# nh2/lz4-frame-conduit

Hardware: AMD Instinct MI355X
Metric: GiB/s end-to-end (compress+decompress), 4 MiB blocks, 1/2/4/8 GPUs vs liblz4 (higher is better)
Workload: dtype u8

## Files before the change

### lz4_frame_conduit_amd/csrc/decode_fused.cuh

```cuda
#pragma once
#include "common.cuh"
#include "decode.cuh"

namespace lz4f {

template <int W> struct FzCfg;
template <> struct FzCfg<8> { static constexpr int WAVES = 8; static constexpr uint32_t STAGE = 8192, RING = 8, LDS_BUDGET = 40960; };
template <> struct FzCfg<4> { static constexpr int WAVES = 4; static constexpr uint32_t STAGE = 2048, RING = 4, LDS_BUDGET = 20480; };
struct FzCfgS8 { static constexpr int WAVES = 8; static constexpr uint32_t STAGE = 4096 - 576, RING = 16, LDS_BUDGET = 40960; };
struct FzCfgS4 { static constexpr int WAVES = 4; static constexpr uint32_t STAGE = 2048, RING = 8, LDS_BUDGET = 20480; };
constexpr uint32_t FZ_OVER = 576;
#ifndef FZ_FED_ROUNDS
#define FZ_FED_ROUNDS 1
#endif
#ifndef FZ_STORE_SC1
#define FZ_STORE_SC1 0
#endif
#ifndef FZ_FED_OCC
#define FZ_FED_OCC 8
#endif
constexpr int      FZ_MATCH_SET = 3;
constexpr uint32_t FZ_SRC_BIAS = 1u << 22;
constexpr uint32_t FZ_PEND = 32;
__device__ __forceinline__ bool fz_wait_expired(uint64_t t0, uint64_t budget) { return __builtin_amdgcn_s_memrealtime() - t0 > budget; }

template <class C>
struct alignas(16) FzShared {
    uint4    ring[C::RING][64];
    uint8_t  stage[2][C::STAGE + FZ_OVER];
    uint4    gt[C::WAVES - 1][2][64];
    uint32_t produced;
    uint32_t total_slots;
    uint32_t last_count;
    uint32_t per_slot;
    uint32_t finished;
    uint32_t match_done;
    uint32_t slot_done[C::RING];
    uint32_t slot_cnt[C::RING];
    uint32_t pend_n, prev_ready, own_front;
    uint32_t wait_lo;
    uint32_t pend_dst[FZ_PEND], pend_len[FZ_PEND], pend_off[FZ_PEND];
    int32_t  status;
    uint32_t out_size;
    uint32_t wait_hi;
};
static_assert(sizeof(FzShared<FzCfg<8>>) <= FzCfg<8>::LDS_BUDGET && sizeof(FzShared<FzCfg<4>>) <= FzCfg<4>::LDS_BUDGET, "workgroups per CU");
static_assert(sizeof(FzShared<FzCfgS8>) <= FzCfgS8::LDS_BUDGET && sizeof(FzShared<FzCfgS4>) <= FzCfgS4::LDS_BUDGET, "workgroups per CU");

__device__ __forceinline__ uint32_t lds_peek(const uint32_t* p) { return __atomic_load_n(p, __ATOMIC_RELAXED); }
__device__ __forceinline__ void lds_poke(uint32_t* p, uint32_t v) { __atomic_store_n(p, v, __ATOMIC_RELAXED); }

template <class C>
__device__ __forceinline__ void fz_stage_issue(uint8_t* slot, const uint8_t* __restrict__ in, uint32_t csize, uint32_t s)
{
    const uint32_t lane = lane_id();
    const uint32_t base = s * C::STAGE;
    if (base >= csize) return;
    const uint32_t end = (base + C::STAGE + FZ_OVER < csize) ? base + C::STAGE + FZ_OVER : csize;
    const uint32_t span = end - base;
    for (uint32_t piece = 0; piece < span; piece += 1024) {
        const uint32_t o = piece + lane * 16;
        if (o + 16 <= span) __builtin_amdgcn_global_load_lds((gptr_t)(in + base + o), (lptr_t)(slot + piece), 16, 0, 0);
    }
    const uint32_t tail0 = span & ~15u;
    if (lane < span - tail0) slot[tail0 + lane] = in[base + tail0 + lane];
}

template <class C>
__device__ __forceinline__ void fz_parser(FzShared<C>& sh, const uint8_t* __restrict__ in, uint32_t csize, uint32_t cap, uint64_t hist,
                                          unsigned long long* prof)
{
#ifdef FZ_PROF
    const unsigned long long t_begin = clock64(); unsigned long long t_ring = 0;
#endif
    const uint32_t lane = lane_id();
    uint8_t* stages = &sh.stage[0][0];
    uint32_t nseq = 0, status = 0;
    uint32_t op = 0;
    int32_t  cur = -1;
    uint32_t d0 = 0, d1 = 0, d2 = 0, d3 = 0;

    if (csize == 0) status = 1;
    else fz_stage_issue<C>(stages, in, csize, 0);
    auto need = [&](uint32_t qq) {
        const int32_t s = (int32_t)(qq / C::STAGE);
        if (s == cur) return;
#pragma unroll 1
        for (int32_t it = (s == cur + 1) ? 1 : 0; it < 2; it++) {
            asm volatile("s_waitcnt vmcnt(0)" ::: "memory");
            fz_stage_issue<C>(stages + (uint32_t)((s + it) & 1) * (C::STAGE + FZ_OVER), in, csize, (uint32_t)(s + it));
        }
        cur = s;
    };
    typedef uint32_t v4u_t __attribute__((ext_vector_type(4)));
    v4u_t win = {0u, 0u, 0u, 0u};
    uint32_t wb = 0xFFFFFC00u;
    auto reload = [&](uint32_t qq) {
        need(qq);
        const uint32_t s = qq / C::STAGE;
        const uint32_t o = (qq - s * C::STAGE) & ~7u;
        const uint32_t addr = (uint32_t)(uintptr_t)(lptr_t)(stages + (s & 1) * (C::STAGE + FZ_OVER)) + o + 8u * lane;
        asm volatile("ds_read2_b64 %0, %1 offset1:1\n\ts_waitcnt lgkmcnt(0)" : "=&v"(win) : "v"(addr) : "memory");
        wb = qq & ~7u;
    };
    auto fetch = [&](uint32_t qq) -> uint64_t {
        uint32_t rel = qq - wb;
        if (rel >= 504u) { reload(qq); rel = qq - wb; }
        const uint32_t l = rel >> 3, sh8 = (rel & 7u) * 8u;
        const uint64_t lo = (uint64_t)(uint32_t)__builtin_amdgcn_readlane(win.x, l) | ((uint64_t)(uint32_t)__builtin_amdgcn_readlane(win.y, l) << 32);
        const uint64_t hi = (uint64_t)(uint32_t)__builtin_amdgcn_readlane(win.z, l) | ((uint64_t)(uint32_t)__builtin_amdgcn_readlane(win.w, l) << 32);
        return (lo >> sh8) | ((hi << 1) << (63u - sh8));
    };
    auto ext_slow = [&](uint32_t pos, uint32_t& after) -> uint32_t {
        uint32_t add = 0;
        for (;;) {
            if (pos >= csize || add > 0x7FFF0000u) { status = 1; after = pos; return add; }
            const uint32_t b = uni((uint32_t)in[pos]);
            add += b; pos++;
            if (b != 255) { after = pos; return add; }
        }
    };
    uint32_t v_src = 0, v_lit = 0, v_op = 0, v_ml = 0;
    const uint32_t plog = csize < (96u << 10) ? 3u : 6u, pmask = (1u << plog) - 1u;
    if (lane == 0) sh.per_slot = pmask + 1;
    const uint32_t hist_reach = hist > 65536 ? 65536u : (uint32_t)hist;
    auto finish_slot = [&](uint32_t count) -> bool {
        uint32_t off = 0;
        bool bad = false;
        if (lane < count) {
            const uint64_t room = (uint64_t)cap - v_op;
            if (v_ml) {
                const uint8_t* q = in + v_src + v_lit;
                off = (uint32_t)q[0] | ((uint32_t)q[1] << 8);
                bad = off == 0 || off > v_op + v_lit + hist_reach || (uint64_t)v_lit + v_ml + 5 > room || (uint64_t)v_lit + 12 > room;
            } else bad = v_lit > room;
        }
        d0 = v_src | ((off & 0xFFu) << 24);
        d1 = v_lit | ((off >> 8) << 24);
        d2 = v_op;
        d3 = v_ml;
        return __ballot(bad) == 0;
    };
    auto publish = [&](uint32_t slot_idx) {
#ifdef FZ_PROF
        const unsigned long long tr = clock64();
#endif
        while (slot_idx >= lds_peek(&sh.match_done) + C::RING) __builtin_amdgcn_s_sleep(8);
#ifdef FZ_PROF
        t_ring += clock64() - tr;
#endif
        sh.ring[slot_idx % C::RING][lane] = uint4{d0, d1, d2, d3};
        asm volatile("s_waitcnt lgkmcnt(0)" ::: "memory");
        lds_poke(&sh.produced, slot_idx + 1);
    };
    auto fetch_byte = [&](uint32_t qq) -> uint32_t {
        uint32_t rel = qq - wb;
        if (rel >= 504u) { reload(qq); rel = qq - wb; }
        const uint32_t l = rel >> 3, sh8 = (rel & 7u) * 8u;
        const uint64_t lo = (uint64_t)(uint32_t)__builtin_amdgcn_readlane(win.x, l) | ((uint64_t)(uint32_t)__builtin_amdgcn_readlane(win.y, l) << 32);
        return (uint32_t)(lo >> sh8) & 0xFFu;
    };

    uint32_t pos = 0;
    uint32_t fin = status;
    while (fin == 0) {
        const uint32_t token = fetch_byte(pos);
        uint32_t lit = token >> 4;
        uint32_t p = pos + 1;
        uint32_t bad = 0;
        if (lit == 15) {
            const uint64_t x = fetch(pos) >> 8;
            const uint32_t f = (uint32_t)__builtin_ctzll(~x);
            const uint32_t k = f >> 3;
            lit = 15u + 255u * k + (uint32_t)((x >> (f & 56u)) & 0xFF);
            p = pos + 2 + k;
            if (k == 7) { lit = 15u + ext_slow(pos + 1, p); bad |= status; }
        }
        bad |= p > csize ? 1u : 0u;
        const uint32_t in_left = csize - p;
        const bool is_last = lit > in_left || lit + 8 > in_left || lit + 12 > cap - op;
        uint32_t mlen = 0, npos = pos;
        if (!is_last) {
            const uint32_t qo = p + lit;
            mlen = token & 15;
            npos = qo + 2;
            if (mlen == 15) {
                const uint64_t x = fetch(qo) >> 16;
                const uint32_t f = (uint32_t)__builtin_ctzll(~x);
                const uint32_t k = f >> 3;
                mlen = 15u + 255u * k + (uint32_t)((x >> (f & 56u)) & 0xFF);
                npos = qo + 3 + k;
                if (k == 6) { mlen = 15u + ext_slow(qo + 2, npos); bad |= status; }
                bad |= npos + 4 >= csize ? 1u : 0u;
            }
            mlen += 4;
            bad |= mlen > cap - (op + lit) ? 1u : 0u;
        } else {
            bad |= lit != in_left ? 1u : 0u;
            bad |= lit > cap - op ? 1u : 0u;
        }
        fin |= bad;
        if (fin == 0) {
            const uint32_t slot = nseq & pmask;
            uint32_t keep;
            asm("s_mov_b32 %4, m0\n\ts_mov_b32 m0, %5\n\tv_writelane_b32 %0, %6, m0\n\tv_writelane_b32 %1, %7, m0\n\tv_writelane_b32 %2, %8, m0\n\tv_writelane_b32 %3, %9, m0\n\ts_mov_b32 m0, %4"
                : "+v"(v_src), "+v"(v_lit), "+v"(v_op), "+v"(v_ml), "=&s"(keep) : "s"(slot), "s"(p), "s"(lit), "s"(op), "s"(mlen));
            nseq++;
            op += lit + mlen;
            if (slot == pmask) {
                if (finish_slot(pmask + 1)) publish((nseq >> plog) - 1);
                else { fin |= 1u; nseq -= pmask + 1; }
            }
            pos = npos;
            fin |= is_last ? 2u : (pos >= csize ? 1u : 0u);
        }
    }
    if ((fin & 1u) == 0 && (nseq & pmask) && !finish_slot(nseq & pmask)) fin |= 1u;
    if (fin & 1u) status = 1;
    const uint32_t full = nseq >> plog, part = (status == 0) ? (nseq & pmask) : 0;
    if (part) {
        while (full >= lds_peek(&sh.match_done) + C::RING) __builtin_amdgcn_s_sleep(8);
        sh.ring[full % C::RING][lane] = uint4{d0, d1, d2, d3};
    }
    sh.total_slots = status ? lds_peek(&sh.produced) : full + (part ? 1u : 0u);
    sh.last_count = part ? part : pmask + 1;
    sh.out_size = op;
    sh.status = status ? -1 : 0;
    asm volatile("s_waitcnt lgkmcnt(0)" ::: "memory");
    lds_poke(&sh.finished, 1u);
    if (part) { asm volatile("s_waitcnt lgkmcnt(0)" ::: "memory"); lds_poke(&sh.produced, full + 1); }
#ifdef FZ_PROF
    if (prof && blockIdx.x == 0 && lane == 0) { prof[0] = clock64() - t_begin; prof[1] = t_ring; prof[2] = nseq; }
#endif
}

template <class C>
__device__ __forceinline__ void fz_feeder(FzShared<C>& sh, const SeqDesc* __restrict__ desc, const uint32_t* __restrict__ dsrc, uint32_t nseq,
                                          uint32_t csize, uint32_t cap, uint64_t hist, uint64_t pay_before)
{
    const uint32_t lane = lane_id();
    uint32_t per = (nseq + (C::WAVES - 1) - 1) / (C::WAVES - 1);
    per = per > 64 ? 64u : (per < 8 ? 8u : per);
    const uint32_t nslots = (nseq + per - 1) / per;
    uint32_t expect = 0, status = nseq ? 0u : 1u, published = 0;
    uint4 nxt = {0u, 0u, 0u, 0u};
    uint32_t nxt_src = 0xFFFFFFFFu;
    if (lane < per && lane < nseq) { nxt = ((const uint4*)desc)[lane]; if (dsrc) nxt_src = dsrc[lane]; }
    for (uint32_t slot = 0; slot < nslots && !status; slot++) {
        const uint32_t first = slot * per;
        const uint32_t count = (nseq - first < per) ? nseq - first : per;
        uint4 d = nxt;
        if (nxt_src < (1u << 23) && !(d.w >> 31) && (d.w & 0xFFFFFFu))
            d = uint4{(d.x & 0xFFFFFFu) | ((nxt_src & 0xFFu) << 24), (d.y & 0xFFFFFFu) | (((nxt_src >> 8) & 0xFFu) << 24), d.z,
                      (d.w & 0xFFFFFFu) | 0x80000000u | ((nxt_src >> 16) << 24)};
        const uint32_t nx = first + per + lane;
        nxt = uint4{0u, 0u, 0u, 0u}; nxt_src = 0xFFFFFFFFu;
        if (lane < per && nx < nseq) { nxt = ((const uint4*)desc)[nx]; if (dsrc) nxt_src = dsrc[nx]; }
        const uint32_t p = d.x & 0xFFFFFFu, lit = d.y & 0xFFFFFFu, op = d.z, ml = d.w & 0xFFFFFFu;
        const bool direct = (d.w >> 31) != 0;
        const uint32_t f24 = (d.x >> 24) | ((d.y >> 24) << 8) | (((d.w >> 24) & 0x7Fu) << 16);
        const uint64_t dm = (uint64_t)op + lit, end = dm + ml;
        const uint32_t prev_end = __shfl_up((uint32_t)end, 1);
        const bool last = first + lane + 1 == nseq;
        bool bad = op != (lane == 0 ? expect : prev_end) || (uint64_t)p + lit > csize || end > cap;
        if (last) bad |= ml != 0 || direct;
        else {
            bad |= ml < 4 || end + 5 > cap;
            const int64_t rel = (int64_t)f24 - (int64_t)FZ_SRC_BIAS;
            bad |= direct ? (rel + (int64_t)ml > (int64_t)csize || -rel > (int64_t)pay_before) : (f24 == 0 || f24 > 65535u || f24 > dm + hist);
        }
        if (__ballot(lane < count && bad)) { status = 1; break; }
        expect = __shfl((uint32_t)end, (int)count - 1);
        while (slot >= lds_peek(&sh.match_done) + C::RING && (int32_t)lds_peek((const uint32_t*)&sh.status) >= 0) __builtin_amdgcn_s_sleep(8);
        if ((int32_t)lds_peek((const uint32_t*)&sh.status) < 0) { status = 1; break; }
        sh.ring[slot % C::RING][lane] = d;
        sh.slot_cnt[slot % C::RING] = count;
        if (slot + 1 == nslots) break;
        asm volatile("s_waitcnt lgkmcnt(0)" ::: "memory");
        lds_poke(&sh.produced, slot + 1);
        published = slot + 1;
    }
    sh.total_slots = status ? published : nslots;
    sh.last_count = status ? 64u : nseq - (nslots - 1) * per;
    sh.out_size = expect;
    sh.status = status ? -1 : 0;
    asm volatile("s_waitcnt lgkmcnt(0)" ::: "memory");
    lds_poke(&sh.finished, 1u);
    if (!status) { asm volatile("s_waitcnt lgkmcnt(0)" ::: "memory"); lds_poke(&sh.produced, nslots); }
}

template <class C, bool FED = false>
__device__ __forceinline__ void fz_copier(FzShared<C>& sh, const uint8_t* __restrict__ in, uint8_t* out, uint32_t cw ,
                                          const uint8_t* safe , unsigned long long* prof, const uint32_t* prev_done = nullptr)
{
    const uint32_t lane = lane_id();
    unsigned long long t_wait_p = 0, t_lit = 0, t_wait_m = 0, t_match = 0, n_slots = 0, t_dep = 0, t_drain = 0;
    auto dump = [&]() { if (prof && FED && lane == 0) { atomicAdd(prof + 76, t_wait_p); atomicAdd(prof + 77, t_lit); atomicAdd(prof + 78, t_wait_m); atomicAdd(prof + 79, t_match); }
                        if (prof && blockIdx.x == 0 && lane == 0) { unsigned long long* o = prof + 8 * (cw + 1); o[0] = t_wait_p; o[1] = t_lit; o[2] = t_wait_m; o[3] = t_match; o[4] = n_slots; o[5] = t_dep; o[6] = t_drain; } };
    for (uint32_t slot = cw;; slot += C::WAVES - 1) {
        const unsigned long long c0 = clock64();
        for (;;) {
            if (lds_peek(&sh.produced) > slot) break;
            if (lds_peek(&sh.finished) && slot >= lds_peek(&sh.total_slots)) { dump(); return; }
            __builtin_amdgcn_s_sleep(4);
        }
        const unsigned long long c1 = clock64(); t_wait_p += c1 - c0; n_slots++;
        __builtin_amdgcn_s_setprio(1);
        const uint4 d = sh.ring[slot % C::RING][lane];
        uint32_t count = FED ? 64u : lds_peek(&sh.per_slot);
        if (FED) count = lds_peek(&sh.slot_cnt[slot % C::RING]);
        else if (lds_peek(&sh.finished) && slot + 1 == lds_peek(&sh.total_slots)) count = lds_peek(&sh.last_count);
        count = uni(count);
        const uint32_t vsrc = d.x & 0xFFFFFFu, vlen = d.y & 0xFFFFFFu, vdst = d.z, vml = FED ? (d.w & 0xFFFFFFu) : d.w, voff = (d.x >> 24) | ((d.y >> 24) << 8);
        const bool vdirect = FED && lane < count && (d.w >> 31) != 0;
        const uint32_t vmsrc = (voff | (((d.w >> 24) & 0x7Fu) << 16)) - FZ_SRC_BIAS;

        {
            uint4* T0 = sh.gt[cw][0];
            uint4* T1 = sh.gt[cw][1];
            const uint32_t L = lane < count ? vlen : 0u, M = vdirect ? vml : 0u;
            auto scan = [&](uint32_t v, uint32_t& total) -> uint32_t {
                uint32_t incl = v;
#pragma unroll
                for (int sft = 1; sft < 64; sft <<= 1) { const uint32_t t = __shfl_up(incl, sft); if ((int)lane >= sft) incl += t; }
                total = __builtin_amdgcn_readlane(incl, 63);
                return incl - v;
            };
            auto find = [&](uint32_t u) -> uint32_t {
                uint32_t j = 0;
#pragma unroll
                for (uint32_t step = 32; step; step >>= 1) { const uint32_t c = j + step; if (T0[c].x <= u) j = c; }
                return j;
            };
            uint32_t total;
            {
                const uint32_t uL = L >= 16 ? (L + 15) >> 4 : 0u, uM = M >= 16 ? (M + 15) >> 4 : 0u;
                const uint32_t P = scan(uL + uM, total);
                if (total) {
                    T0[lane] = uint4{P, uL, L, M};
                    T1[lane] = uint4{vsrc, vmsrc, vdst, 0u};
                    __builtin_amdgcn_fence(__ATOMIC_RELEASE, "wavefront"); __builtin_amdgcn_wave_barrier();
                }
            }
            if (total) {
                auto ld = [&](Piece& pc, uint32_t u, uint32_t& dof, bool& act) {
                    const uint32_t j = find(u);
                    const uint4 e0 = T0[j], e1 = T1[j];
                    uint32_t r = u - e0.x;
                    const bool isM = r >= e0.y;
                    r -= isM ? e0.y : 0u;
                    const uint32_t len = isM ? e0.w : e0.z;
                    uint32_t off = r * 16u;
                    off = (off + 16u > len) ? len - 16u : off;
                    act = u < total;
                    dof = e1.z + (isM ? e0.z : 0u) + off;
                    const uint8_t* a = act ? in + (int32_t)((isM ? e1.y : e1.x) + off) : safe;
                    const v4u_ua t = *(const v4u_ua*)a;
                    pc.a = t.a; pc.b = t.b; pc.c = t.c; pc.d = t.d;
                };
                typedef uint32_t u32x4 __attribute__((ext_vector_type(4)));
                typedef u32x4 u32x4_ua __attribute__((aligned(1)));
                auto st = [&](const Piece& pc, uint32_t dof, bool act) {
                    if (!act) return;
#if FZ_STORE_SC1 == 1
                    if (FED) { const u32x4 v = u32x4{pc.a, pc.b, pc.c, pc.d}; uint8_t* q = out + dof; asm volatile("global_store_dwordx4 %0, %1, off sc1\n\ts_nop 1" :: "v"(q), "v"(v) : "memory"); }
#elif FZ_STORE_SC1 == 2
                    if (FED) { const u32x4 v = u32x4{pc.a, pc.b, pc.c, pc.d}; uint8_t* q = out + dof; asm volatile("global_store_dwordx4 %0, %1, off sc0 sc1\n\ts_nop 1" :: "v"(q), "v"(v) : "memory"); }
#elif FZ_STORE_SC1 == 3
                    if (FED) *(v4u_ua*)(out + dof) = v4u_ua{pc.a, pc.b, pc.c, pc.d};
#else
                    if (FED) __builtin_nontemporal_store(u32x4{pc.a, pc.b, pc.c, pc.d}, (u32x4_ua*)(out + dof));
#endif
                    else *(v4u_ua*)(out + dof) = v4u_ua{pc.a, pc.b, pc.c, pc.d};
                };
                constexpr int G = FED ? FZ_FED_ROUNDS : 1;
                Piece pa[G], pb[G];
                uint32_t da[G], db[G];
                bool xa[G], xb[G];
                uint32_t base = 0;
#pragma unroll
                for (int i = 0; i < G; i++) ld(pa[i], base + 64 * i + lane, da[i], xa[i]);
                base += 64 * G;
                for (;;) {
                    const bool more_b = base < total;
#pragma unroll
                    for (int i = 0; i < G; i++) ld(pb[i], base + 64 * i + lane, db[i], xb[i]);
                    base += 64 * G;
#pragma unroll
                    for (int i = 0; i < G; i++) st(pa[i], da[i], xa[i]);
                    if (!more_b) break;
                    const bool more_a = base < total;
#pragma unroll
                    for (int i = 0; i < G; i++) ld(pa[i], base + 64 * i + lane, da[i], xa[i]);
                    base += 64 * G;
#pragma unroll
                    for (int i = 0; i < G; i++) st(pb[i], db[i], xb[i]);
                    if (!more_a) break;
                }
            }
            uint32_t total_b;
            {
                const uint32_t bL = L < 16 ? L : 0u, bM = M < 16 ? M : 0u;
                const uint32_t P = scan(bL + bM, total_b);
                if (total_b) {
                    T0[lane] = uint4{P, bL, L, M};
                    T1[lane] = uint4{vsrc, vmsrc, vdst, 0u};
                    __builtin_amdgcn_fence(__ATOMIC_RELEASE, "wavefront"); __builtin_amdgcn_wave_barrier();
                }
            }
            for (uint32_t base = 0; base < total_b; base += 128) {
                uint8_t v[2]; uint32_t dof[2]; bool act[2];
#pragma unroll
                for (int i = 0; i < 2; i++) {
                    const uint32_t u = base + 64 * i + lane;
                    const uint32_t j = find(u);
                    const uint4 e0 = T0[j], e1 = T1[j];
                    uint32_t r = u - e0.x;
                    const bool isM = r >= e0.y;
                    r -= isM ? e0.y : 0u;
                    act[i] = u < total_b;
                    dof[i] = e1.z + (isM ? e0.z : 0u) + r;
                    const uint8_t* a = act[i] ? in + (int32_t)((isM ? e1.y : e1.x) + r) : safe;
                    v[i] = *a;
                }
#pragma unroll
                for (int i = 0; i < 2; i++) if (act[i]) out[dof[i]] = v[i];
            }
        }
        const unsigned long long c2 = clock64(); t_lit += c2 - c1;
        __builtin_amdgcn_s_setprio(0);
        const uint64_t on_chain = __ballot(lane < count && vml != 0 && !vdirect);
        if (on_chain) {
            while (lds_peek(&sh.match_done) < slot) {
                if ((int32_t)lds_peek((const uint32_t*)&sh.status) < 0) { dump(); return; }
                __builtin_amdgcn_s_sleep(2);
            }
        }
        __builtin_amdgcn_sched_barrier(0); const unsigned long long c3 = clock64(); t_wait_m += c3 - c2; __builtin_amdgcn_sched_barrier(0);
        __builtin_amdgcn_s_setprio(2);
        if (on_chain) {
            constexpr int NJ = FZ_MATCH_SET;
            const uint32_t mdm = vdst + vlen;
            const int32_t ms0 = (int32_t)mdm - (int32_t)voff, ms1 = ms0 + (int32_t)vml;
            const bool has = lane < count && vml != 0 && !vdirect;
            const uint64_t fastmask = __ballot(has && vml >= 16 && vml <= 1024 && voff >= vml);
            uint64_t todo = __ballot(has), unstored = todo;
            uint32_t dep_lo = 0, dep_hi = 0;
            for (uint64_t mm = todo; mm; mm &= mm - 1) {
                const uint32_t k = (uint32_t)__builtin_ctzll(mm);
                const uint32_t dk = __builtin_amdgcn_readlane(mdm, k), mk = __builtin_amdgcn_readlane(vml, k);
                const bool dep = k < lane && ms0 < (int32_t)(dk + mk) && ms1 > (int32_t)dk;
                if (k < 32) dep_lo |= dep ? (1u << k) : 0u; else dep_hi |= dep ? (1u << (k - 32)) : 0u;
            }
            __builtin_amdgcn_sched_barrier(0); t_dep += clock64() - c3; __builtin_amdgcn_sched_barrier(0);
            if (FED && prev_done && lds_peek(&sh.prev_ready) && __ballot(has && ms0 < 0)) __builtin_amdgcn_fence(__ATOMIC_ACQUIRE, "agent");
            if (FED && prev_done && !lds_peek(&sh.prev_ready)) {
                const uint32_t np = lds_peek(&sh.pend_n);
                bool defer = has && ms0 < -(int32_t)lds_peek(&sh.own_front);
                for (uint32_t q = 0; q < np; q++) {
                    const int32_t lo = (int32_t)sh.pend_dst[q], hi = lo + (int32_t)sh.pend_len[q];
                    defer |= has && ms0 < hi && ms1 > lo;
                }
                uint64_t dmask = __ballot(defer);
                while (dmask) {
                    const bool more = has && !defer && (((dep_lo & (uint32_t)dmask) | (dep_hi & (uint32_t)(dmask >> 32))) != 0);
                    const uint64_t add = __ballot(more);
                    if (!add) break;
                    defer |= more; dmask |= add;
                }
                if (dmask) {
                    const uint32_t cnt = (uint32_t)__builtin_popcountll(dmask);
                    if (np + cnt > FZ_PEND) {
                        uint32_t v = 0;
                        const uint64_t budget = (uint64_t)lds_peek(&sh.wait_lo) | ((uint64_t)lds_peek(&sh.wait_hi) << 32);
                        for (const uint64_t t0 = __builtin_amdgcn_s_memrealtime();;) {
                            v = __hip_atomic_load(prev_done, __ATOMIC_RELAXED, __HIP_MEMORY_SCOPE_AGENT);
                            if (v == 1u || v == 2u || fz_wait_expired(t0, budget)) break;
                            __builtin_amdgcn_s_sleep(8);
                        }
                        __builtin_amdgcn_fence(__ATOMIC_ACQUIRE, "agent");
                        if (v != 1u) { lds_poke((uint32_t*)&sh.status, 0xFFFFFFFFu); dump(); return; }
                        for (uint32_t q = 0; q < np; q++) wave_copy_match(out + (int32_t)sh.pend_dst[q], sh.pend_off[q], sh.pend_len[q]);
                        asm volatile("s_waitcnt vmcnt(0)" ::: "memory");
                        lds_poke(&sh.pend_n, 0u);
                        lds_poke(&sh.prev_ready, 1u);
                    } else {
                        if (defer) {
                            const uint32_t at = np + (uint32_t)__builtin_popcountll(dmask & ((1ull << lane) - 1ull));
                            sh.pend_dst[at] = mdm; sh.pend_len[at] = vml; sh.pend_off[at] = voff;
                        }
                        asm volatile("s_waitcnt lgkmcnt(0)" ::: "memory");
                        lds_poke(&sh.pend_n, np + cnt);
                        todo &= ~dmask; unstored &= ~dmask;
                    }
                }
            }
            auto ready = [&]() -> uint64_t {
                return __ballot(has && ((dep_lo & (uint32_t)unstored) | (dep_hi & (uint32_t)(unstored >> 32))) == 0) & todo;
            };
            auto select = [&](CopyJob (&J)[NJ], uint64_t rf) -> uint64_t {
                uint64_t taken = 0;
#pragma unroll
                for (int i = 0; i < NJ; i++) {
                    J[i] = CopyJob{safe, out, 0};
                    if (rf) {
                        const uint32_t c = (uint32_t)__builtin_ctzll(rf);
                        rf &= rf - 1; taken |= 1ull << c;
                        const uint32_t dm = __builtin_amdgcn_readlane(mdm, c);
                        J[i] = CopyJob{out + dm - __builtin_amdgcn_readlane(voff, c), out + dm, (uint32_t)__builtin_amdgcn_readlane(vml, c)};
                    }
                }
                todo &= ~taken;
                return taken;
            };
            while (todo) {
                uint64_t r = ready();
                if ((r & fastmask) == 0) {
                    const uint32_t c = (uint32_t)__builtin_ctzll(r);
                    wave_copy_match(out + __builtin_amdgcn_readlane(mdm, c), __builtin_amdgcn_readlane(voff, c), __builtin_amdgcn_readlane(vml, c));
                    todo &= ~(1ull << c); unstored &= ~(1ull << c);
                    continue;
                }
                CopyJob A[NJ], B[NJ];
                Piece PA[NJ], PB[NJ];
                uint64_t ma = select(A, r & fastmask), mb;
#pragma unroll
                for (int i = 0; i < NJ; i++) job_load(PA[i], A[i], safe);
                for (;;) {
                    mb = select(B, ready() & fastmask);
#pragma unroll
                    for (int i = 0; i < NJ; i++) job_load(PB[i], B[i], safe);
#pragma unroll
                    for (int i = 0; i < NJ; i++) job_store(A[i], PA[i]);
                    unstored &= ~ma;
                    if (mb == 0) break;
                    ma = select(A, ready() & fastmask);
#pragma unroll
                    for (int i = 0; i < NJ; i++) job_load(PA[i], A[i], safe);
#pragma unroll
                    for (int i = 0; i < NJ; i++) job_store(B[i], PB[i]);
                    unstored &= ~mb;
                    if (ma == 0) break;
                }
            }
        }
        __builtin_amdgcn_sched_barrier(0);
        const unsigned long long c5 = clock64();
        __builtin_amdgcn_sched_barrier(0);
        asm volatile("s_waitcnt vmcnt(0)" ::: "memory");
        __builtin_amdgcn_sched_barrier(0);
        t_drain += clock64() - c5;
        __builtin_amdgcn_sched_barrier(0);
        lds_poke(&sh.slot_done[slot % C::RING], slot + 1);
        asm volatile("s_waitcnt lgkmcnt(0)" ::: "memory");
        for (;;) {
            const uint32_t md = lds_peek(&sh.match_done);
            if (lds_peek(&sh.slot_done[md % C::RING]) != md + 1) break;
            if (lane == 0) atomicCAS(&sh.match_done, md, md + 1);
            asm volatile("s_waitcnt lgkmcnt(0)" ::: "memory");
        }
        __builtin_amdgcn_s_setprio(0);
        t_match += clock64() - c3;
    }
}

template <class C, bool FED = false>
__device__ __forceinline__ int32_t fz_decode_block(FzShared<C>& sh, const uint8_t* __restrict__ in, uint32_t csize, uint8_t* out, uint32_t cap, uint64_t hist,
                                                   const uint8_t* safe, unsigned long long* prof, const SeqDesc* __restrict__ fed = nullptr, uint32_t nfed = 0,
                                                   const uint32_t* __restrict__ fed_src = nullptr, uint64_t pay_before = 0, const uint32_t* prev_done = nullptr,
                                                   uint32_t own_front = 0, bool first_of_group = true)
{
    const uint32_t wave = uni(threadIdx.x >> 6);
    __syncthreads();
    if (threadIdx.x == 0) { sh.produced = 0; sh.total_slots = 0; sh.last_count = 64; sh.finished = 0; sh.match_done = 0; sh.status = 0; sh.out_size = 0; }
    if (threadIdx.x < C::RING) sh.slot_done[threadIdx.x] = 0;
    if (threadIdx.x == 0) { if (first_of_group) { sh.pend_n = 0; sh.prev_ready = 0; } sh.own_front = own_front; }
    __syncthreads();
    if (wave == 0) {
        __builtin_amdgcn_s_setprio(3);
        if (FED) fz_feeder<C>(sh, fed, fed_src, nfed, csize, cap, hist, pay_before);
        else fz_parser<C>(sh, in, csize, cap, hist, prof);
        __builtin_amdgcn_s_setprio(0);
    }
    else fz_copier<C, FED>(sh, in, out, wave - 1, safe, prof, prev_done);
    __syncthreads();
    const int32_t st = (int32_t)uni((uint32_t)sh.status);
    const uint32_t osz = uni(sh.out_size);
    return st < 0 ? -1 : (int32_t)osz;
}

template <class C>
__global__ __launch_bounds__(64 * C::WAVES, 8) void k_decode_blocks_fused(const uint8_t* __restrict__ frame, uint8_t* dst, uint64_t dst_cap,
                                                                          BlockOut* __restrict__ table, const ResultRec* __restrict__ res,
                                                                          uint32_t n_max, uint32_t linked, uint32_t block_size, uint64_t hist0,
                                                                          unsigned long long* prof, const uint32_t* __restrict__ only_if)
{
    __shared__ FzShared<C> sh;
    if (res->status != ST_OK) return;
    if (only_if && *only_if == 0) return;
    const uint32_t n = res->n_blocks < n_max ? res->n_blocks : n_max;
    const uint32_t tid = threadIdx.x;
    if (linked && blockIdx.x != 0) return;
    uint32_t b = linked ? 0u : blockIdx.x;
    const uint32_t b_end = linked ? n : (b < n ? b + 1 : b);
    uint64_t out = 0;
    for (; b < b_end; b++) {
        const BlockOut e = table[b];
        const uint32_t csz = e.word & 0x7FFFFFFFu;
        const uint64_t at = linked ? out : e.dst_off;
        const uint32_t room = linked ? (uint32_t)((dst_cap - out < block_size) ? dst_cap - out : block_size) : e.dst_size;
        int32_t got;
        if (e.word >> 31) {
            if (csz > room) got = -2;
            else {
                const uint32_t per = (((csz + C::WAVES - 1) / C::WAVES) + 15) & ~15u;
                const uint32_t a = (tid >> 6) * per;
                if (a < csz) wave_copy_disjoint(dst + at + a, frame + e.src_off + a, (csz - a < per) ? csz - a : per);
                got = (int32_t)csz;
            }
        } else {
            got = fz_decode_block<C>(sh, frame + e.src_off, csz, dst + at, room, linked ? out + hist0 : 0, frame, prof);
        }
        if (tid == 0) { table[b].dst_off = at; table[b].dst_size = (uint32_t)got; }
        if (got < 0) {
            if (linked) for (uint32_t k = b + 1 + tid; k < n; k += 64 * C::WAVES) table[k].dst_size = 0;
            break;
        }
        out += (uint32_t)got;
        __syncthreads();
    }
}

}
```

Measured before the change: 757.6.

## Replace binary-search piece lookup with LDS scatter plus DPP max-scan, rotate pipeline

```diff
diff --git a/lz4_frame_conduit_amd/csrc/decode_fused.cuh b/lz4_frame_conduit_amd/csrc/decode_fused.cuh
--- a/lz4_frame_conduit_amd/csrc/decode_fused.cuh
+++ b/lz4_frame_conduit_amd/csrc/decode_fused.cuh
@@ -10,8 +10,8 @@
 struct FzCfgS8 { static constexpr int WAVES = 8; static constexpr uint32_t STAGE = 4096 - 576, RING = 16, LDS_BUDGET = 40960; };
 struct FzCfgS4 { static constexpr int WAVES = 4; static constexpr uint32_t STAGE = 2048, RING = 8, LDS_BUDGET = 20480; };
 constexpr uint32_t FZ_OVER = 576;
-#ifndef FZ_FED_ROUNDS
-#define FZ_FED_ROUNDS 1
+#ifndef FZ_FED_SETS
+#define FZ_FED_SETS 2
 #endif
 #ifndef FZ_STORE_SC1
 #define FZ_STORE_SC1 0
@@ -43,6 +43,7 @@
     int32_t  status;
     uint32_t out_size;
     uint32_t wait_hi;
+    uint32_t dump[C::WAVES - 1];
 };
 static_assert(sizeof(FzShared<FzCfg<8>>) <= FzCfg<8>::LDS_BUDGET && sizeof(FzShared<FzCfg<4>>) <= FzCfg<4>::LDS_BUDGET, "workgroups per CU");
 static_assert(sizeof(FzShared<FzCfgS8>) <= FzCfgS8::LDS_BUDGET && sizeof(FzShared<FzCfgS4>) <= FzCfgS4::LDS_BUDGET, "workgroups per CU");
@@ -326,25 +327,42 @@
                 total = __builtin_amdgcn_readlane(incl, 63);
                 return incl - v;
             };
-            auto find = [&](uint32_t u) -> uint32_t {
-                uint32_t j = 0;
-#pragma unroll
-                for (uint32_t step = 32; step; step >>= 1) { const uint32_t c = j + step; if (T0[c].x <= u) j = c; }
-                return j;
+            auto lookup = [&](uint32_t base, uint32_t P, uint32_t& carry) -> uint32_t {
+                const uint32_t at = P - base;
+                T1[lane].w = 0u;
+                uint32_t* q = at < 64u ? &T1[at].w : &sh.dump[cw];
+                *q = lane + 1u;
+                __builtin_amdgcn_fence(__ATOMIC_RELEASE, "wavefront"); __builtin_amdgcn_wave_barrier(); __builtin_amdgcn_fence(__ATOMIC_ACQUIRE, "wavefront");
+                uint32_t v = T1[lane].w, t;
+                t = (uint32_t)__builtin_amdgcn_update_dpp(0, (int)v, 0x111 , 0xf, 0xf, false); v = t > v ? t : v;
+                t = (uint32_t)__builtin_amdgcn_update_dpp(0, (int)v, 0x112 , 0xf, 0xf, false); v = t > v ? t : v;
+                t = (uint32_t)__builtin_amdgcn_update_dpp(0, (int)v, 0x114 , 0xf, 0xf, false); v = t > v ? t : v;
+                t = (uint32_t)__builtin_amdgcn_update_dpp(0, (int)v, 0x118 , 0xf, 0xf, false); v = t > v ? t : v;
+                t = (uint32_t)__builtin_amdgcn_update_dpp(0, (int)v, 0x142 , 0xa, 0xf, false); v = t > v ? t : v;
+                t = (uint32_t)__builtin_amdgcn_update_dpp(0, (int)v, 0x143 , 0xc, 0xf, false); v = t > v ? t : v;
+                v = v > carry ? v : carry;
+                carry = (uint32_t)__builtin_amdgcn_readlane((int)v, 63);
+                __builtin_amdgcn_fence(__ATOMIC_RELEASE, "wavefront"); __builtin_amdgcn_wave_barrier();
+                return v - 1u;
             };
             uint32_t total;
-            {
-                const uint32_t uL = L >= 16 ? (L + 15) >> 4 : 0u, uM = M >= 16 ? (M + 15) >> 4 : 0u;
-                const uint32_t P = scan(uL + uM, total);
-                if (total) {
-                    T0[lane] = uint4{P, uL, L, M};
-                    T1[lane] = uint4{vsrc, vmsrc, vdst, 0u};
-                    __builtin_amdgcn_fence(__ATOMIC_RELEASE, "wavefront"); __builtin_amdgcn_wave_barrier();
-                }
-            }
+            const uint32_t uL = L >= 16 ? (L + 15) >> 4 : 0u, nA = uL + (M >= 16 ? (M + 15) >> 4 : 0u);
+            const uint32_t PA = scan(nA, total);
             if (total) {
-                auto ld = [&](Piece& pc, uint32_t u, uint32_t& dof, bool& act) {
-                    const uint32_t j = find(u);
+                T0[lane] = uint4{PA, uL, L, M};
+                T1[lane] = uint4{vsrc, vmsrc, vdst, 0u};
+                __builtin_amdgcn_fence(__ATOMIC_RELEASE, "wavefront"); __builtin_amdgcn_wave_barrier();
+            }
+            if (total) {
+                uint32_t carry = 0;
+                typedef uint32_t u32x4 __attribute__((ext_vector_type(4)));
+                typedef u32x4 u32x4_ua __attribute__((aligned(1)));
+                typedef const __attribute__((address_space(1))) uint8_t* gbytes_t;
+                const gbytes_t gin = (gbytes_t)((uint64_t)uni((uint32_t)(uintptr_t)in) | ((uint64_t)uni((uint32_t)((uintptr_t)in >> 32)) << 32));
+                auto ld = [&](Piece& pc, uint32_t base, uint32_t& dof) {
+                    const uint32_t j = lookup(base, nA ? PA : 0xFFFFFFFFu, carry);
+                    uint32_t u = base + lane;
+                    u = u < total ? u : total - 1;
                     const uint4 e0 = T0[j], e1 = T1[j];
                     uint32_t r = u - e0.x;
                     const bool isM = r >= e0.y;
@@ -352,16 +370,11 @@
                     const uint32_t len = isM ? e0.w : e0.z;
                     uint32_t off = r * 16u;
                     off = (off + 16u > len) ? len - 16u : off;
-                    act = u < total;
                     dof = e1.z + (isM ? e0.z : 0u) + off;
-                    const uint8_t* a = act ? in + (int32_t)((isM ? e1.y : e1.x) + off) : safe;
-                    const v4u_ua t = *(const v4u_ua*)a;
-                    pc.a = t.a; pc.b = t.b; pc.c = t.c; pc.d = t.d;
+                    const u32x4 t = *(const __attribute__((address_space(1))) u32x4_ua*)(gin + (int32_t)((isM ? e1.y : e1.x) + off));
+                    pc.a = t.x; pc.b = t.y; pc.c = t.z; pc.d = t.w;
                 };
-                typedef uint32_t u32x4 __attribute__((ext_vector_type(4)));
-                typedef u32x4 u32x4_ua __attribute__((aligned(1)));
-                auto st = [&](const Piece& pc, uint32_t dof, bool act) {
-                    if (!act) return;
+                auto st = [&](const Piece& pc, uint32_t dof) {
 #if FZ_STORE_SC1 == 1
                     if (FED) { const u32x4 v = u32x4{pc.a, pc.b, pc.c, pc.d}; uint8_t* q = out + dof; asm volatile("global_store_dwordx4 %0, %1, off sc1\n\ts_nop 1" :: "v"(q), "v"(v) : "memory"); }
 #elif FZ_STORE_SC1 == 2
@@ -373,47 +386,47 @@
 #endif
                     else *(v4u_ua*)(out + dof) = v4u_ua{pc.a, pc.b, pc.c, pc.d};
                 };
-                constexpr int G = FED ? FZ_FED_ROUNDS : 1;
-                Piece pa[G], pb[G];
-                uint32_t da[G], db[G];
-                bool xa[G], xb[G];
-                uint32_t base = 0;
-#pragma unroll
-                for (int i = 0; i < G; i++) ld(pa[i], base + 64 * i + lane, da[i], xa[i]);
-                base += 64 * G;
-                for (;;) {
-                    const bool more_b = base < total;
-#pragma unroll
-                    for (int i = 0; i < G; i++) ld(pb[i], base + 64 * i + lane, db[i], xb[i]);
-                    base += 64 * G;
-#pragma unroll
-                    for (int i = 0; i < G; i++) st(pa[i], da[i], xa[i]);
-                    if (!more_b) break;
-                    const bool more_a = base < total;
-#pragma unroll
-                    for (int i = 0; i < G; i++) ld(pa[i], base + 64 * i + lane, da[i], xa[i]);
-                    base += 64 * G;
-#pragma unroll
-                    for (int i = 0; i < G; i++) st(pb[i], db[i], xb[i]);
-                    if (!more_a) break;
+                constexpr int D = FED ? FZ_FED_SETS : 2;
+                Piece ps[D];
+                uint32_t dp[D];
+                const uint32_t rounds = (total + 63) >> 6;
+#pragma unroll
+                for (int k = 0; k < D - 1; k++) ld(ps[k], 64 * k, dp[k]);
+                const uint32_t left = rounds > D - 1 ? rounds - (D - 1) : 0u, rem = left % D;
+                uint32_t base = 64 * (D - 1);
+                auto trip = [&]() {
+#pragma unroll
+                    for (int k = 0; k < D; k++) {
+                        ld(ps[(k + D - 1) % D], base + 64 * k, dp[(k + D - 1) % D]);
+                        __builtin_amdgcn_sched_barrier(0);
+                        st(ps[k], dp[k]);
+                        __builtin_amdgcn_sched_barrier(0);
+                    }
+                    base += 64 * D;
+                };
+                uint32_t trips = left / D;
+                if (trips) { trip(); while (--trips) trip(); }
+#pragma unroll
+                for (int k = 0; k < 2 * D - 2; k++) {
+                    if ((uint32_t)k < rem) ld(ps[(k + D - 1) % D], base + 64 * k, dp[(k + D - 1) % D]);
+                    if ((uint32_t)k < rem + D - 1) st(ps[k % D], dp[k % D]);
                 }
             }
             uint32_t total_b;
-            {
-                const uint32_t bL = L < 16 ? L : 0u, bM = M < 16 ? M : 0u;
-                const uint32_t P = scan(bL + bM, total_b);
-                if (total_b) {
-                    T0[lane] = uint4{P, bL, L, M};
-                    T1[lane] = uint4{vsrc, vmsrc, vdst, 0u};
-                    __builtin_amdgcn_fence(__ATOMIC_RELEASE, "wavefront"); __builtin_amdgcn_wave_barrier();
-                }
-            }
+            const uint32_t bL = L < 16 ? L : 0u, nB = bL + (M < 16 ? M : 0u);
+            const uint32_t PB = scan(nB, total_b);
+            if (total_b) {
+                T0[lane] = uint4{PB, bL, L, M};
+                T1[lane] = uint4{vsrc, vmsrc, vdst, 0u};
+                __builtin_amdgcn_fence(__ATOMIC_RELEASE, "wavefront"); __builtin_amdgcn_wave_barrier();
+            }
+            uint32_t carry_b = 0;
             for (uint32_t base = 0; base < total_b; base += 128) {
                 uint8_t v[2]; uint32_t dof[2]; bool act[2];
 #pragma unroll
                 for (int i = 0; i < 2; i++) {
                     const uint32_t u = base + 64 * i + lane;
-                    const uint32_t j = find(u);
+                    const uint32_t j = lookup(base + 64 * i, nB ? PB : 0xFFFFFFFFu, carry_b);
                     const uint4 e0 = T0[j], e1 = T1[j];
                     uint32_t r = u - e0.x;
                     const bool isM = r >= e0.y;
```

Result: slower. 745.6 (-1.6%).
